# srv902/FOCUS

Measured on AMD Instinct MI355X. Metric: clips/sec (fwd+bwd+opt step) ORViT-MF 16x224, higher is better.
Workload: dtype bf16; 1 GPU; ORViT-Motionformer 16x224, 4 objects, batch=8 per GPU (BASELINE configs[1]); global_batch=8, frames=16, crop=224, objects=4, parallelism=dp1, optimizer=adamw+clipnorm

## Files before the change

### focus_amd/csrc/traj_time2_gw.hip

```cpp
#include "focus_common.h"
#include <algorithm>

namespace {

typedef __attribute__((ext_vector_type(8))) __bf16 bf16x8;
typedef __attribute__((ext_vector_type(4))) short s16x4;
typedef __attribute__((ext_vector_type(4))) float f32x4;
typedef __attribute__((address_space(3))) s16x4 lds_s16x4;

constexpr int HD = 64, TR = 32;
constexpr int C_ = 768;
constexpr int NSUB = C_ / 128;
constexpr int GT_BYTES = TR * C_ * 2, QT_BYTES = TR * HD * 2, STAGE = GT_BYTES + QT_BYTES;

union Frag { bf16x8 v; s16x4 t[2]; uint4 u; };

__device__ __forceinline__ int offb(int row, int ch) { return 256 * row + 16 * (ch ^ (((row & 3) << 2) | ((row >> 2) & 3))); }

__device__ __forceinline__ bf16x8 tr_frag_g(const char* sub, int r0, int c0, int lane) {
    const int i = lane & 15, q = i >> 2, p = i & 3;
    const int ch = (c0 >> 3) + (p >> 1), bo = 8 * (p & 1);
    Frag f;
    f.t[0] = __builtin_amdgcn_ds_read_tr16_b64_v4i16((lds_s16x4*)(sub + offb(r0 + q, ch) + bo));
    f.t[1] = __builtin_amdgcn_ds_read_tr16_b64_v4i16((lds_s16x4*)(sub + offb(r0 + 4 + q, ch) + bo));
    return f.v;
}
__device__ __forceinline__ bf16x8 tr_frag_q(const char* qt, int r0, int c0, int lane) {
    const int i = lane & 15, q = i >> 2, p = i & 3;
    const int o = (c0 + 4 * p) * 2;
    Frag f;
    f.t[0] = __builtin_amdgcn_ds_read_tr16_b64_v4i16((lds_s16x4*)(qt + (r0 + q) * 128 + o));
    f.t[1] = __builtin_amdgcn_ds_read_tr16_b64_v4i16((lds_s16x4*)(qt + (r0 + 4 + q) * 128 + o));
    return f.v;
}

__global__ __launch_bounds__(512) void time2_gw_kernel(const bf16_t* __restrict__ g, const bf16_t* __restrict__ q2,
                                                       const bf16_t* __restrict__ wk, int64_t wk_ld, bf16_t* __restrict__ dq2,
                                                       float* __restrict__ slabs, int R, int heads, int tiles_per_split) {
    extern __shared__ __attribute__((aligned(1024))) char smem[];
    const int h = blockIdx.y, sp = blockIdx.x;
    const int tid = threadIdx.x, lane = tid & 63, w = __builtin_amdgcn_readfirstlane(tid >> 6);
    const int ntiles_all = R / TR;
    const int t_begin = sp * tiles_per_split, t_end = min(ntiles_all, t_begin + tiles_per_split);
    const int row16_ = lane & 15, kq_ = lane >> 4;
    const int mb = w & 1, nbq = w >> 1;
    const bf16_t* gh = g + (int64_t)h * R * C_;

    bf16x8 wf[C_ / 32];
    {
        const bf16_t* wrow = wk + (int64_t)(h * HD + nbq * 16 + row16_) * wk_ld + kq_ * 8;
#pragma unroll
        for (int ks = 0; ks < C_ / 32; ++ks) wf[ks] = *reinterpret_cast<const bf16x8*>(wrow + ks * 32);
    }
    f32x4 accw[4][6];
#pragma unroll
    for (int a = 0; a < 4; ++a)
#pragma unroll
        for (int j = 0; j < 6; ++j) accw[a][j] = (f32x4){0.f, 0.f, 0.f, 0.f};
    asm volatile("s_waitcnt vmcnt(0)" ::: "memory");
#pragma unroll
    for (int ks = 0; ks < C_ / 32; ++ks) asm volatile("" : "+v"(wf[ks]));

    const uint32_t sm_a = lds_addr_of(smem);
    auto dma = [&](int t, int st) __attribute__((always_inline)) {
        const int64_t r0 = (int64_t)t * TR;
        const uint32_t base = sm_a + st * STAGE;
#pragma unroll
        for (int j = 0; j < 6; ++j) {
            const int p = w * 6 + j, sub = p >> 3, rg = p & 7;
            const int row = rg * 4 + (lane >> 4), pos = lane & 15;
            const int ch = pos ^ (((row & 3) << 2) | ((row >> 2) & 3));
            glds16(gh + (r0 + row) * C_ + sub * 128 + ch * 8, __builtin_amdgcn_readfirstlane(base + sub * 8192 + rg * 1024));
        }
        if (w < 4) {
            const int row = w * 8 + (lane >> 3);
            glds16(q2 + (r0 + row) * (int64_t)(heads * HD) + h * HD + (lane & 7) * 8,
                   __builtin_amdgcn_readfirstlane(base + GT_BYTES + w * 1024));
        }
    };
    if (t_begin >= t_end) return;
    dma(t_begin, 0);
    int st = 0;
    for (int t = t_begin; t < t_end; ++t) {
        const bool more = t + 1 < t_end;
        if (more) dma(t + 1, st ^ 1);
        if (more) { if (w < 4) asm volatile("s_waitcnt vmcnt(7)" ::: "memory"); else asm volatile("s_waitcnt vmcnt(6)" ::: "memory"); }
        else asm volatile("s_waitcnt vmcnt(0)" ::: "memory");
        __builtin_amdgcn_s_barrier();
        const char* gt = smem + st * STAGE;
        const char* qt = gt + GT_BYTES;
        int lane_o = lane;
        asm volatile("" : "+v"(lane_o));
        const int row16 = lane_o & 15, kq = lane_o >> 4;
        f32x4 accq = {0.f, 0.f, 0.f, 0.f};
#pragma unroll
        for (int ks = 0; ks < C_ / 32; ++ks) {
            const int col = ks * 32 + kq * 8;
            const bf16x8 af = *reinterpret_cast<const bf16x8*>(gt + (col >> 7) * 8192 + offb(mb * 16 + row16, (col & 127) >> 3));
            accq = __builtin_amdgcn_mfma_f32_16x16x32_bf16(af, wf[ks], accq, 0, 0, 0);
        }
        {
            bf16_t* o = dq2 + ((int64_t)t * TR + mb * 16 + kq * 4) * (heads * HD) + h * HD + nbq * 16 + row16;
#pragma unroll
            for (int r = 0; r < 4; ++r) o[(int64_t)r * (heads * HD)] = f32_to_bf16(accq[r]);
        }
#pragma unroll
        for (int j = 0; j < 6; ++j) {
            const int c = w * 96 + j * 16;
            const bf16x8 gb = tr_frag_g(gt + (c >> 7) * 8192, 8 * kq, c & 127, lane_o);
#pragma unroll
            for (int a = 0; a < 4; ++a) {
                const bf16x8 qa = tr_frag_q(qt, 8 * kq, a * 16, lane_o);
                accw[a][j] = __builtin_amdgcn_mfma_f32_16x16x32_bf16(qa, gb, accw[a][j], 0, 0, 0);
            }
        }
        asm volatile("s_waitcnt lgkmcnt(0)" ::: "memory");
        __builtin_amdgcn_s_barrier();
        st ^= 1;
    }
    float* out = slabs + ((int64_t)sp * heads * HD + h * HD) * C_;
#pragma unroll
    for (int a = 0; a < 4; ++a)
#pragma unroll
        for (int j = 0; j < 6; ++j)
#pragma unroll
            for (int r = 0; r < 4; ++r) out[(int64_t)(a * 16 + kq_ * 4 + r) * C_ + w * 96 + j * 16 + row16_] = accw[a][j][r];
}

__global__ __launch_bounds__(256) void time2_gw_reduce_kernel(const float* __restrict__ slabs, float* __restrict__ dwk, int64_t n4,
                                                              int splits) {
    const int64_t i = (int64_t)blockIdx.x * 256 + threadIdx.x;
    if (i >= n4) return;
    float4 s = reinterpret_cast<const float4*>(slabs)[i];
#pragma unroll 4
    for (int k = 1; k < splits; ++k) {
        const float4 v = reinterpret_cast<const float4*>(slabs)[(int64_t)k * n4 + i];
        s.x += v.x; s.y += v.y; s.z += v.z; s.w += v.w;
    }
    reinterpret_cast<float4*>(dwk)[i] = s;
}

int gw_splits(int R, int heads) {
    const int tiles = R / TR;
    return std::max(1, std::min(tiles, 256 / std::max(heads, 1)));
}

}

extern "C" int focus_traj_time2_gw_ok(int R, int heads, int d, int dtype) {
    return dtype == FOCUS_BF16 && d == HD && heads * d == C_ && R >= TR && R % TR == 0;
}

extern "C" size_t focus_traj_time2_gw_workspace_bytes(int R, int heads, int d) {
    if (!focus_traj_time2_gw_ok(R, heads, d, FOCUS_BF16)) return 0;
    return (size_t)gw_splits(R, heads) * C_ * C_ * sizeof(float);
}

extern "C" int focus_traj_time2_gw(const void* g, const void* q2, const void* wk, int64_t wk_ld, void* dq2, float* dwk, void* ws,
                                   size_t ws_bytes, int R, int heads, int d, int dtype, void* stream) {
    if (!g || !q2 || !wk || !dq2 || !dwk || !ws) return FOCUS_ERR_NULL;
    if (!focus_traj_time2_gw_ok(R, heads, d, dtype) || (wk_ld & 7)) return FOCUS_ERR_SHAPE;
    if (!focus_aligned(g, 16) || !focus_aligned(q2, 16) || !focus_aligned(wk, 16) || !focus_aligned(dwk, 16)) return FOCUS_ERR_ALIGN;
    if (ws_bytes < focus_traj_time2_gw_workspace_bytes(R, heads, d)) return FOCUS_ERR_WORKSPACE;
    hipStream_t s = static_cast<hipStream_t>(stream);
    const int splits = gw_splits(R, heads), tiles = R / TR;
    const int tps = (tiles + splits - 1) / splits;
    const int used = (tiles + tps - 1) / tps;
    auto k = time2_gw_kernel;
    const size_t lds = 2 * (size_t)STAGE;
    static bool once = (hipFuncSetAttribute((const void*)k, hipFuncAttributeMaxDynamicSharedMemorySize, lds) == hipSuccess);
    (void)once;
    hipLaunchKernelGGL(k, dim3(used, heads), dim3(512), lds, s, (const bf16_t*)g, (const bf16_t*)q2, (const bf16_t*)wk, wk_ld,
                       (bf16_t*)dq2, (float*)ws, R, heads, tps);
    FOCUS_CHECK_LAUNCH();
    const int64_t n4 = (int64_t)C_ * C_ / 4;
    hipLaunchKernelGGL(time2_gw_reduce_kernel, dim3((unsigned)cdiv64(n4, 256)), dim3(256), 0, s, (const float*)ws, dwk, n4, used);
    FOCUS_CHECK_LAUNCH();
    return FOCUS_OK;
}
```

### focus_amd/ops.py

```python
import ctypes
import weakref

import torch

from . import _lib
from ._lib import BF16, F32, GemmDesc

EPI_NONE, EPI_GELU, EPI_RELU, EPI_TANH = _lib.EPI_NONE, _lib.EPI_GELU, _lib.EPI_RELU, _lib.EPI_TANH
_DEPI = {EPI_GELU: _lib.EPI_DGELU, EPI_RELU: _lib.EPI_DRELU, EPI_TANH: _lib.EPI_DTANH}


def _dt(t):
    if t.dtype == torch.float32:
        return F32
    if t.dtype == torch.bfloat16:
        return BF16
    raise RuntimeError("focus_amd: unsupported dtype %s (float32 or bfloat16)" % t.dtype)


def _need_gpu(*ts):
    for t in ts:
        if t is not None and not t.is_cuda:
            raise RuntimeError("focus_amd: the hot path runs on the MI355X only (got a %s tensor); "
                               "there is no CPU fallback" % t.device)
# ... 1157 lines not shown
    def backward(ctx, dxt, dxdiag, dcls):
        qkv, xt, cls_out, lse, cls_lse = ctx.saved_tensors
        B, F_, P, heads, d = ctx.dims
        dxt, dxdiag, dcls = dxt.contiguous(), dxdiag.contiguous(), dcls.contiguous()
        dqkv = torch.empty_like(qkv)
        L = _lib.lib()
        nb = L.focus_traj_space_workspace_bytes(B, F_, P, heads, d, _dt(qkv), 1)
        ws = torch.empty(max(nb, 16), device=qkv.device, dtype=torch.uint8)
        _lib.check(L.focus_traj_space_bwd(_p(qkv), _p(xt), _p(cls_out), _p(lse), _p(cls_lse), _p(dxt), _p(dxdiag),
                                          _p(dcls), _p(dqkv), _p(ws), nb, B, F_, P, heads, d, _dt(qkv), _stream()),
                   "traj_space_bwd")
        return dqkv, None, None, None


def traj_space(qkv, F_, P, heads):
    return _TrajSpaceFn.apply(qkv, F_, P, heads)


class _TrajTimeFn(torch.autograd.Function):
    @staticmethod
    def forward(ctx, q2, k2, xt, heads):
        _need_gpu(q2, k2, xt)
        q2, k2, xt = q2.contiguous(), k2.contiguous(), xt.contiguous()
        B, S, F_, C = xt.shape
        d = C // heads
        out = torch.empty(B, S, C, device=xt.device, dtype=xt.dtype)
        attn2 = torch.empty(B, heads, S, F_, device=xt.device, dtype=torch.float32)
        _lib.check(_lib.lib().focus_traj_time_fwd(_p(q2), _p(k2), _p(xt), _p(out), S * C, _p(attn2), B, S, F_, heads, d,
                                                  _dt(xt), _stream()), "traj_time_fwd")
        ctx.save_for_backward(q2, k2, xt, attn2)
        ctx.heads = heads
        return out

    @staticmethod
    def backward(ctx, dout):
        q2, k2, xt, attn2 = ctx.saved_tensors
        B, S, F_, C = xt.shape
        dout = dout.contiguous()
        dq2, dk2, dxt = torch.empty_like(q2), torch.empty_like(k2), torch.empty_like(xt)
        _lib.check(_lib.lib().focus_traj_time_bwd(_p(q2), _p(k2), _p(xt), _p(attn2), _p(dout), S * C, _p(dq2), _p(dk2),
                                                  _p(dxt), 0, B, S, F_, ctx.heads, C // ctx.heads, _dt(xt),
                                                  _stream()), "traj_time_bwd")
        return dq2, dk2, dxt, None


def traj_time(q2, k2, xt, heads):
    return _TrajTimeFn.apply(q2, k2, xt, heads)


class _TrajTimeBlockFn(torch.autograd.Function):

    @staticmethod
    def forward(ctx, q2, xt, w_kv, b_kv, cls_out, heads):
        _need_gpu(q2, xt, w_kv)
        q2, xt = q2.contiguous(), xt.contiguous()
        B, S, F_, C = xt.shape
        d = C // heads
        wk = shadow(w_kv, xt.dtype)[:C]
        bk = b_kv.detach()[:C] if b_kv is not None else None
        k2 = mm_nt(xt.view(-1, C), wk, bias=bk).view(B, S, F_, C)
        out = torch.empty(B, S + 1, C, device=xt.device, dtype=xt.dtype)
        out[:, 0].copy_(cls_out.reshape(B, C))
        attn2 = torch.empty(B, heads, S, F_, device=xt.device, dtype=torch.float32)
        _lib.check(_lib.lib().focus_traj_time_fwd(_p(q2), _p(k2), _p(xt), _p(out, C), (S + 1) * C, _p(attn2), B, S, F_,
                                                  heads, d, _dt(xt), _stream()), "traj_time_fwd")
        ctx.save_for_backward(q2, k2, xt, attn2, w_kv)
        ctx.heads, ctx.has_b, ctx.cls_shape = heads, b_kv is not None, cls_out.shape
        return out

    @staticmethod
    def backward(ctx, dcat):
        q2, k2, xt, attn2, w_kv = ctx.saved_tensors
        B, S, F_, C = xt.shape
        dcat = dcat.contiguous()
        dq2, dk2, dxt_a = torch.empty_like(q2), torch.empty_like(k2), torch.empty_like(xt)
        _lib.check(_lib.lib().focus_traj_time_bwd(_p(q2), _p(k2), _p(xt), _p(attn2), _p(dcat, C), (S + 1) * C, _p(dq2),
                                                  _p(dk2), _p(dxt_a), 0, B, S, F_, ctx.heads, C // ctx.heads, _dt(xt),
                                                  _stream()), "traj_time_bwd")
        dk2f, xt2 = dk2.view(-1, C), xt.view(-1, C)
        dw = db = dwk = dbk = None
        join = None
        if ctx.needs_input_grad[2]:
            dwk, dbk, join = wgrad_async(dk2f, xt2, ctx.has_b and ctx.needs_input_grad[3])
        dxt = None
        if ctx.needs_input_grad[1]:
            if xt.dtype == torch.bfloat16 and C % 64 == 0:
                wt = shadow(w_kv, xt.dtype, transposed=True)
                dxt = mm_nt(dk2f, wt[:, :C], residual=dxt_a.view(-1, C))
            else:
                dxt = mm_nn(dk2f, shadow(w_kv, xt.dtype)[:C]).add_(dxt_a.view(-1, C))
            dxt = dxt.view(B, S, F_, C)
        if join is not None:
            join()
        if dwk is not None:
            dw = torch.empty(2 * C, C, device=xt.device, dtype=torch.float32)
            dw[:C].copy_(dwk)
            dw[C:].zero_()
            if dbk is not None:
                db = torch.zeros(2 * C, device=xt.device, dtype=torch.float32)
                db[:C].copy_(dbk)
        dcls = dcat[:, :1].reshape(ctx.cls_shape) if ctx.needs_input_grad[4] else None
        return dq2, dxt, dw, db, dcls, None


def traj_time_block(q2, xt, w_kv, b_kv, cls_out, heads):
    return _TrajTimeBlockFn.apply(q2, xt, w_kv, b_kv, cls_out, heads)


class _TrajTime2BlockFn(torch.autograd.Function):

    @staticmethod
    def forward(ctx, q2, xt, w_kv, b_kv, cls_out, heads):
        _need_gpu(q2, xt, w_kv)
        q2, xt = q2.contiguous(), xt.contiguous()
        B, S, F_, C = xt.shape
        d = C // heads
        L = _lib.lib()
        wkT = shadow(w_kv, xt.dtype, transposed=True)
        out = torch.empty(B, S + 1, C, device=xt.device, dtype=xt.dtype)
        out[:, 0].copy_(cls_out.reshape(B, C))
        attn2 = torch.empty(B, S, heads, F_, device=xt.device, dtype=torch.float32)
        nb = L.focus_traj_time2_workspace_bytes(B, S, F_, heads, d)
        ws = torch.empty(nb // 4, device=xt.device, dtype=torch.float32)
        _lib.check(L.focus_traj_time2_fwd(_p(q2), _p(xt), _p(wkT), wkT.stride(0), _p(out, C), (S + 1) * C, _p(attn2),
                                          _p(ws), nb, B, S, F_, heads, d, _dt(xt), _stream()), "traj_time2_fwd")
        ctx.save_for_backward(q2, xt, attn2, w_kv)
        ctx.heads, ctx.has_b, ctx.cls_shape = heads, b_kv is not None, cls_out.shape
        return out

    @staticmethod
    def backward(ctx, dcat):
        q2, xt, attn2, w_kv = ctx.saved_tensors
        heads = ctx.heads
        B, S, F_, C = xt.shape
        d = C // heads
        dev = xt.device
        L = _lib.lib()
        dcat = dcat.contiguous()
        wkT = shadow(w_kv, xt.dtype, transposed=True)
        dxt = torch.empty_like(xt)
        g = torch.empty(heads, B * S, C, device=dev, dtype=xt.dtype)
        dl = torch.empty(B, S, F_, 16, device=dev, dtype=xt.dtype)
        _lib.check(L.focus_traj_time2_bwd(_p(q2), _p(xt), _p(wkT), wkT.stride(0), _p(attn2), _p(dcat, C), (S + 1) * C,
                                          _p(dxt), _p(g), _p(dl), B, S, F_, heads, d, _dt(xt), _stream()), "traj_time2_bwd")
        R = B * S
        dq2 = dw = db = None
        if (ctx.needs_input_grad[0] and ctx.needs_input_grad[2] and L.focus_traj_time2_gw_ok(R, heads, d, _dt(xt))
                and _os.environ.get("FOCUS_TIME2_GW", "1") != "0"):
            wk = shadow(w_kv, xt.dtype)
            dq2 = torch.empty(B, S, C, device=dev, dtype=xt.dtype)
            dw = torch.empty(2 * C, C, device=dev, dtype=torch.float32)
            nbw = L.focus_traj_time2_gw_workspace_bytes(R, heads, d)
            wsw = torch.empty(nbw // 4, device=dev, dtype=torch.float32)
            _lib.check(L.focus_traj_time2_gw(_p(g), _p(q2), _p(wk), wk.stride(0), _p(dq2), _p(dw), _p(wsw), nbw, R, heads, d,
                                             _dt(xt), _stream()), "traj_time2_gw")
            dw[C:].zero_()
            if ctx.has_b and ctx.needs_input_grad[3]:
                db = torch.zeros(2 * C, device=dev, dtype=torch.float32)
            dcls = dcat[:, :1].reshape(ctx.cls_shape) if ctx.needs_input_grad[4] else None
            return dq2, dxt, dw, db, dcls, None
        if ctx.needs_input_grad[0]:
            wk = shadow(w_kv, xt.dtype)
            dq2 = torch.empty(B, S, C, device=dev, dtype=xt.dtype)
            gemm(R, d, C, (g, 0), (C, 1, 0, R * C), (wk, 0), (1, C, 0, d * C), (dq2, 0), (C, 1, 0, d),
                 batch=(1, heads))
        if ctx.needs_input_grad[2]:
            dw = torch.empty(2 * C, C, device=dev, dtype=torch.float32)
            nbw = L.focus_gemm_tn_batched_workspace_bytes(d, C, R, heads)
            wsw = torch.empty(max(nbw, 16) // 4, device=dev, dtype=torch.float32)
            gemm(d, C, R, (q2, 0), (1, C, 0, d), (g, 0), (C, 1, 0, R * C), (dw, 0), (C, 1, 0, d * C),
                 batch=(1, heads), aux=(wsw, 0))
            dw[C:].zero_()
            if ctx.has_b and ctx.needs_input_grad[3]:
                db = torch.zeros(2 * C, device=dev, dtype=torch.float32)
        dcls = dcat[:, :1].reshape(ctx.cls_shape) if ctx.needs_input_grad[4] else None
        return dq2, dxt, dw, db, dcls, None


def traj_time2_ok(xt, heads):
    if _os.environ.get("FOCUS_TIME2", "1") == "0" or xt.dtype != torch.bfloat16:
        return False
    B, S, F_, C = xt.shape
    return C % heads == 0 and C // heads == 64 and heads <= 16 and F_ in (4, 8, 16)


def traj_time2_block(q2, xt, w_kv, b_kv, cls_out, heads):
    return _TrajTime2BlockFn.apply(q2, xt, w_kv, b_kv, cls_out, heads)


class _SmallAttnFn(torch.autograd.Function):

    @staticmethod
    def forward(ctx, q, k, v, heads, scale, causal, drop):
        _need_gpu(q, k, v)
        B, N, C = q.shape
        M = k.shape[1]
        d = C // heads
        dev, dt = q.device, q.dtype
        att = torch.empty(B, heads, N, M, device=dev, dtype=dt)
        L = _lib.lib()
        ctx.heads, ctx.scale = heads, scale

        def rows_ok(t):
            return t.stride(2) == 1 and t.stride(0) == t.shape[1] * t.stride(1) and t.stride(1) >= C

        ctx.fused = (not causal and drop is None and bool(L.focus_small_attn_ok(N, M, d))
                     and rows_ok(q) and rows_ok(k) and rows_ok(v))
        if ctx.fused:
            out = torch.empty(B, N, C, device=dev, dtype=dt)
            _lib.check(L.focus_small_attn_fwd(_p(q), _p(k), _p(v), q.stride(1), k.stride(1), v.stride(1), _p(att), _p(out), B,
                                              heads, N, M, d, scale, _dt(q), _stream()), "small_attn_fwd")
            ctx.save_for_backward(q, k, v, att, None)
            return out
        q, k, v = q.contiguous(), k.contiguous(), v.contiguous()
        sa = (M, 1, heads * N * M, N * M)
        gemm(N, M, d, (q, 0), (C, 1, N * C, d), (k, 0), (1, C, M * C, d), (att, 0), sa, batch=(B, heads))
        if causal:
            assert N == M, "causal self-attention"
            _lib.check(L.focus_softmax_causal_fwd(_p(att), _p(att), B * heads * N, M, M, N, scale, _dt(att), _stream()),
                       "softmax_causal_fwd")
        else:
            _lib.check(L.focus_softmax_fwd(_p(att), _p(att), B * heads * N, M, M, scale, _dt(att), _stream()),
                       "softmax_fwd")
        attd = att if drop is None else att * drop
        out = torch.empty(B, N, C, device=dev, dtype=dt)
        gemm(N, d, M, (attd, 0), sa, (v, 0), (C, 1, M * C, d), (out, 0), (C, 1, N * C, d), batch=(B, heads))
        ctx.save_for_backward(q, k, v, att, drop)
        return out

    @staticmethod
    def backward(ctx, dout):
        q, k, v, att, drop = ctx.saved_tensors
        heads, scale = ctx.heads, ctx.scale
        B, N, C = q.shape
        M = k.shape[1]
        d = C // heads
        dout = dout.contiguous()
        if ctx.fused:
            es = q.element_size()
            if (N == M and q.stride(1) == 3 * C == k.stride(1) == v.stride(1) and k.data_ptr() == q.data_ptr() + C * es
                    and v.data_ptr() == k.data_ptr() + C * es):
                dqkv = torch.empty(B, N, 3 * C, device=q.device, dtype=q.dtype)
                dq, dk, dv = dqkv[..., :C], dqkv[..., C:2 * C], dqkv[..., 2 * C:]
            else:
                dq = torch.empty(q.shape, device=q.device, dtype=q.dtype)
                dk = torch.empty(k.shape, device=q.device, dtype=q.dtype)
                dv = torch.empty(v.shape, device=q.device, dtype=q.dtype)
                if not (q.is_contiguous() and k.is_contiguous() and v.is_contiguous()):
                    q, k, v = q.contiguous(), k.contiguous(), v.contiguous()
            _lib.check(_lib.lib().focus_small_attn_bwd(_p(q), _p(k), _p(v), q.stride(1), k.stride(1), v.stride(1), _p(att),
                                                       _p(dout), _p(dq), _p(dk), _p(dv), B, heads, N, M, d, scale, _dt(q),
                                                       _stream()), "small_attn_bwd")
            return dq, dk, dv, None, None, None, None
        sa = (M, 1, heads * N * M, N * M)
        sat = (1, M, heads * N * M, N * M)
        sq = (C, 1, N * C, d)
        sk = (C, 1, M * C, d)
        attd = att if drop is None else att * drop
        datt = torch.empty_like(att)
        gemm(N, M, d, (dout, 0), sq, (v, 0), (1, C, M * C, d), (datt, 0), sa, batch=(B, heads))
        dv = torch.empty_like(v)
        gemm(M, d, N, (attd, 0), sat, (dout, 0), sq, (dv, 0), sk, batch=(B, heads))
        if drop is not None:
            datt = datt * drop
        _lib.check(_lib.lib().focus_softmax_bwd(_p(datt), _p(att), _p(datt), B * heads * N, M, M, scale, _dt(att),
                                                _stream()), "softmax_bwd")
        dq, dk = torch.empty_like(q), torch.empty_like(k)
        gemm(N, d, M, (datt, 0), sa, (k, 0), sk, (dq, 0), sq, batch=(B, heads))
        gemm(M, d, N, (datt, 0), sat, (q, 0), sq, (dk, 0), sk, batch=(B, heads))
        return dq, dk, dv, None, None, None, None


def flash_ok(q, k, v, heads, causal):
    if not (q.is_cuda and q.dtype == torch.bfloat16 and k.dtype == q.dtype and v.dtype == q.dtype and q.dim() == 3):
        return False
    C = q.shape[2]
    if C % heads:
        return False
    for t in (q, k, v):
        if t.stride(2) != 1 or t.stride(1) % 8 or t.stride(0) % 8 or t.data_ptr() % 16:
            return False
    return bool(_lib.lib().focus_flash_attn_ok(q.shape[1], k.shape[1], C // heads, _lib.BF16, int(bool(causal))))


def drop_threshold(p):
    thr = int(round(float(p) * 65536.0))
    assert 0 <= thr < 65536, "dropout probability out of range"
    return thr


def _flash_args(q, k, v, out, lse, heads, scale, causal, thr, seed):
    B, Nq, C = q.shape
    a = _lib.FlashArgs()
    a.q, a.k, a.v, a.out, a.lse = _p(q), _p(k), _p(v), _p(out), _p(lse)
    a.seed = _p(seed) if seed is not None else None
    a.ldq, a.ldk, a.ldv, a.ldo = q.stride(1), k.stride(1), v.stride(1), out.stride(1)
    a.bsq, a.bsk, a.bsv, a.bso = q.stride(0), k.stride(0), v.stride(0), out.stride(0)
    a.B, a.heads, a.Nq, a.Nk, a.d, a.dtype, a.causal = B, heads, Nq, k.shape[1], C // heads, _lib.BF16, int(bool(causal))
    a.drop_thr, a.scale = thr, scale
    return a


class _FlashAttnFn(torch.autograd.Function):

    @staticmethod
    def forward(ctx, q, k, v, heads, scale, causal, thr, seed):
        _need_gpu(q, k, v)
        B, Nq, C = q.shape
        out = torch.empty(B, Nq, C, device=q.device, dtype=q.dtype)
        lse = torch.empty(B, heads, Nq, device=q.device, dtype=torch.float32)
        a = _flash_args(q, k, v, out, lse, heads, scale, causal, thr, seed)
# ... 989 lines not shown
```

### include/focus_amd.h

```cpp
#ifndef FOCUS_AMD_H
#define FOCUS_AMD_H

#include <stddef.h>
#include <stdint.h>

#ifdef __cplusplus
extern "C" {
#endif

enum focus_dtype { FOCUS_F32 = 0, FOCUS_BF16 = 1, FOCUS_FP8_E4M3 = 2  };

enum focus_status {
    FOCUS_OK = 0,
    FOCUS_ERR_SHAPE = -1,
    FOCUS_ERR_DTYPE = -2,
    FOCUS_ERR_ALIGN = -3,
    FOCUS_ERR_LAUNCH = -4,
    FOCUS_ERR_NULL = -5,
    FOCUS_ERR_WORKSPACE = -6
};

const char* focus_strerror(int status);
int focus_abi_version(void);

// ... 102 lines not shown

int focus_roi_align_fwd(const void* feat, int64_t img_stride, int imgs_per_batch, int64_t batch_stride,
                        const float* rois, const int32_t* roi_img, void* out, int NI, int C, int H, int W, int K,
                        int PH, int PW, float spatial_scale, int sampling_ratio, int aligned, int relu, int dtype,
                        void* stream);
size_t focus_roi_align_bwd_workspace_bytes(int NI, int C, int H, int W, int PH, int PW);
int focus_roi_align_bwd(const void* dout, const void* relu_out, const float* rois, const int32_t* roi_img, void* dfeat, int64_t img_stride,
                        int imgs_per_batch, int64_t batch_stride, void* ws, size_t ws_bytes, int NI, int C, int H, int W, int K, int PH, int PW, float spatial_scale,
                        int sampling_ratio, int aligned, int dtype, void* stream);
int focus_roi_align_indices(const float* rois, int32_t* grid, int32_t* nbr, int H, int W, int K, int PH,
                            int PW, float spatial_scale, int sampling_ratio, int aligned, void* stream);

int focus_cell_amax_fwd(const void* x, void* y, int32_t* arg, int K, int cells, int C, int dtype,
                        void* stream);
int focus_cell_amax_bwd(const void* dy, const int32_t* arg, void* dx, int K, int cells, int C, int dtype,
                        void* stream);

int focus_orvit_assemble(const void* x, const void* obj, void* all, int B, int T, int HW, int O, int C, int dtype,
                         void* stream);
int focus_orvit_assemble_bwd(const void* dall, void* dx, void* dobj, int B, int T, int HW, int O, int C, int dtype,
                             void* stream);
int focus_orvit_merge(const void* x, const void* y, const void* mm, const float* scale, void* out, int B, int T, int HW,
                      int O, int C, int dtype, void* stream);
int focus_orvit_merge_bwd(const void* dout, const float* scale, void* dy, void* dmm, int B, int T, int HW, int O, int C,
                          int dtype, void* stream);

int focus_box_layout_fwd(const void* vecs, const float* boxes, void* out, int NF, int O, int C, int H,
                         int W, int dtype, void* stream);
int focus_box_layout_bwd(const void* dout, const float* boxes, void* dvecs, int NF, int O, int C, int H,
                         int W, int dtype, void* stream);

size_t focus_slot_attn_workspace_bytes(int B, int N, int K, int D);
int focus_slot_attn_fwd(const void* k_t, const void* v_t, int64_t kv_bstride, const void* q, void* attn_vis,
                        int64_t attn_bstride, void* upd, float* colsum, void* partial, size_t partial_bytes,
                        int B, int N, int K, int D, float eps, int dtype, void* stream);
int focus_slot_attn_bwd(const void* k_t, const void* v_t, int64_t kv_bstride, const void* q,
                        const void* attn_vis, int64_t attn_bstride, const float* colsum, const void* upd,
                        const void* dupd,
                        const void* dattn_vis, void* dk_t, void* dv_t, int accumulate, void* dq, void* partial,
                        size_t partial_bytes, int B, int N, int K, int D, float eps, int dtype, void* wl, void* stream);
int focus_slot_kv_grad_ok(int K, int D, int dtype, int iters);
int focus_slot_kv_grad(const void* wl0, const void* wl1, const void* wl2, const void* wl3, const void* q0, const void* q1,
                       const void* q2, const void* q3, const void* du0, const void* du1, const void* du2, const void* du3,
                       int iters, void* dk_t, void* dv_t, int64_t kv_bstride, int64_t kv_ld, int B, int N, int K, int D,
                       int dtype, void* stream);

int focus_small_attn_ok(int N, int M, int d);
int focus_small_attn_fwd(const void* q, const void* k, const void* v, int64_t ldq, int64_t ldk, int64_t ldv, void* att,
                         void* out, int B, int heads, int N, int M, int d, float scale, int dtype, void* stream);
int focus_small_attn_bwd(const void* q, const void* k, const void* v, int64_t ldq, int64_t ldk, int64_t ldv, const void* att,
                         const void* dout, void* dq, void* dk, void* dv, int B, int heads, int N, int M, int d, float scale,
                         int dtype, void* stream);

int focus_gru_gates_fwd(void* gi, void* gh, const void* h, void* hn, const float* b_ih, const float* b_hh, int R, int D,
                        int dtype, void* stream);
int focus_gru_gates_bwd(const void* gi, const void* gh, const void* h, const void* dhn, void* dgi, void* dgh,
                        void* dh, void* zero_out, int R, int D, int dtype, void* stream);

int focus_im2col_patches(const float* x, void* cols, int B, int Cin, int T, int H, int W, int kt, int kh,
                         int kw, int dtype, void* stream);

int focus_embed_assemble(const void* patch, const float* cls, const float* pos, const float* temp,
                         void* tokens, int B, int T, int P, int C, int dtype, void* stream);

int focus_xent_ls(const float* logits, const int64_t* target, float* loss_rows, float* dlogits, int R,
                  int Ncls, float smoothing, void* stream);

int focus_transpose_pad(const void* src, int src_dtype, int64_t src_ld, int64_t src_bstride, void* dst,
                        int dst_dtype, int64_t dst_ld, int64_t dst_bstride, int R, int Cc, int batch,
                        void* stream);

typedef struct focus_shadow_item {
    const float* src; void* dst; void* dstT;
    int32_t rows, cols;
} focus_shadow_item;
int focus_shadow_refresh(const focus_shadow_item* items, int n_items, int max_rows, int max_cols, void* stream);

typedef struct focus_adamw_item {
    float* p; float* m; float* v; void* dst; void* dstT;
    int32_t rows, cols, group, unit0, tile_mode, pad_;
} focus_adamw_item;
int focus_adamw_units(int rows, int cols, int tile_mode);
size_t focus_adamw_workspace_bytes(void);
int focus_adamw_step(const focus_adamw_item* items, float* const* grads, int n_items, int n_units, const float* groups, float* steps,
                     void* workspace, size_t workspace_bytes, float* total_norm, double beta1, double beta2, float eps,
                     float max_norm, int write_clipped_grads, void* stream);

typedef struct focus_fp8_item {
    const float* src; void* dst; void* dstT; float* scale;
    int32_t rows, cols;
} focus_fp8_item;
int focus_fp8_refresh(const focus_fp8_item* items, int n_items, int max_rows, int max_cols, void* amax_scratch, void* stream);

typedef struct focus_wgrad_item {
    const void* dy; const void* x; float* dw; float* db;
    int64_t ld_dy, ld_x;
    int32_t M, N, K, pad_;
} focus_wgrad_item;
int focus_linear_wgrad_group_units(const focus_wgrad_item* items, int n_items);
int focus_linear_wgrad_group_plan(const focus_wgrad_item* items, int n_items, void* host_units, size_t bytes);
int focus_linear_wgrad_group(const focus_wgrad_item* items, int n_items, const void* dev_units, void* stream);

typedef struct focus_slot_tail_args {
    int32_t R, D, H, do_gru, do_mlp, do_q;
    float ln1_eps, ln2_eps;
    const void* upd; const void* h;
    const void* w_ih; const void* w_hh; const float* b_ih; const float* b_hh;
    const float* ln1_g; const float* ln1_b; const void* w1; const float* b1; const void* w2; const float* b2;
    const float* ln2_g; const float* ln2_b; const void* wq;
    void* g; void* hn; void* y; float* mean1; float* rstd1; void* a; void* s;
    void* sn; float* mean2; float* rstd2; void* q;
} focus_slot_tail_args;
int focus_slot_tail_ok(int D, int H, int dtype);
int focus_slot_tail_fwd(const focus_slot_tail_args* args, void* stream);
typedef struct focus_slot_tail_bwd_args {
    int32_t R, D, H, do_gru, do_mlp, do_q;
    const void* dout; const void* dq;
    const void* h; const void* g; const void* hn; const void* a; const void* cur;
    const float* mean1; const float* rstd1; const float* mean2; const float* rstd2;
    const float* ln1_g; const float* ln2_g;
    const void* w_ih_t; const void* w_hh_t; const void* w1_t; const void* w2_t; const void* wq_t;
    void* dupd; void* dh; void* ds; void* dz; void* dg; float* part1; float* part2;
    void* ws_dsn; void* ws_dy1; void* ws_res;
} focus_slot_tail_bwd_args;
int focus_slot_tail_bwd_blocks(int R);
int focus_slot_tail_bwd(const focus_slot_tail_bwd_args* args, void* stream);

typedef struct focus_flash_args {
    const void* q; const void* k; const void* v; void* out; float* lse;
    const void* dout; float* delta; void* dq; void* dk; void* dv;
    const uint32_t* seed;
    int64_t ldq, ldk, ldv, ldo, lddo, lddq, lddk, lddv;
    int64_t bsq, bsk, bsv, bso, bsdo, bsdq, bsdk, bsdv;
    int32_t B, heads, Nq, Nk, d, dtype, causal;
    uint32_t drop_thr;
    float scale;
    int32_t pad_;
} focus_flash_args;
int focus_flash_attn_ok(int Nq, int Nk, int d, int dtype, int causal);
int focus_flash_attn_fwd(const focus_flash_args* args, void* stream);
int focus_flash_attn_bwd(const focus_flash_args* args, void* stream);

int focus_decode_attn_ok(int Lmax, int d, int dtype);
int focus_decode_attn(const void* q, int64_t ldq, const void* k_new, const void* v_new, int64_t ldn, void* k_cache,
                      void* v_cache, int64_t ldc, int64_t bsc, void* out, int64_t ldo, int B, int heads, int d, int len,
                      int Lmax, float scale, int dtype, void* stream);
int focus_greedy_next(const void* logits, int64_t ldl, const float* dict, const float* pe_row, int64_t* tok,
                      int64_t tok_stride, void* x_next, int64_t ldx, int B, int V, int D, int dtype, void* stream);

int focus_traj_time2_gw_ok(int R, int heads, int d, int dtype);
size_t focus_traj_time2_gw_workspace_bytes(int R, int heads, int d);
int focus_traj_time2_gw(const void* g, const void* q2, const void* wk, int64_t wk_ld, void* dq2, float* dwk, void* ws,
                        size_t ws_bytes, int R, int heads, int d, int dtype, void* stream);

int focus_rows_ok(int64_t R, int V, int dtype);
int focus_gumbel_fwd(const void* x, const float* e_soft, const float* e_hard, const void* seed, void* z, int64_t* target,
                     float* stats, int64_t R, int V, float tau, int hard, int dtype, int dtype_z, void* stream);
int focus_gumbel_bwd(const void* x, const float* e_soft, const void* seed, const float* stats, const void* dz, void* dx,
                     int64_t R, int V, float tau, int dtype, int dtype_z, void* stream);

int focus_xent_rows_fwd(const void* logits, const int64_t* target, float* loss_rows, float* lse, int64_t R, int V,
                        float smoothing, int dtype, void* stream);
int focus_xent_rows_bwd(const void* logits, const int64_t* target, const float* lse, const float* g, void* dlogits,
                        int64_t R, int V, float smoothing, int dtype, void* stream);

int focus_dropout_add(const void* y, const void* res, const void* seed, int thr, void* out, int64_t n, int dtype,
                      void* stream);

int focus_diag_gather(const void* xt, void* xdiag, int B, int S, int F, int C, int dtype, void* stream);
int focus_diag_scatter_add(const void* dxdiag, void* dxt, int B, int S, int F, int C, int dtype, void* stream);

int focus_scale_add(const void* x, const void* y, const float* scale, float keep, void* out, int B, int64_t per,
                    int dtype, void* stream);

int focus_cast(const void* src, int src_dtype, void* dst, int dst_dtype, int64_t n, void* stream);

#ifdef __cplusplus
}
#endif
#endif
```

Before: 285.9 clips/s.

## Split dq K-reduction across waves via LDS and fuse dW/db zeroing into reduce

The time2 grad-weight kernel now splits the dq2 GEMM over two K halves per wave pair, keeping half the weight fragments in registers. Partial sums go to an LDS buffer and are reduced and stored as vectorized bf16 by the other waves one tile later. MFMA and LDS reads are interleaved with sched_group_barriers, and the q fragments are hoisted out of the dW loop. A new _full entry point makes the reduce kernel also zero the second half of dW and the bias gradient, replacing two separate torch zero launches, at the cost of extra LDS, an extra lgkmcnt wait per tile, and more complex synchronization.

```diff
diff --git a/focus_amd/csrc/traj_time2_gw.hip b/focus_amd/csrc/traj_time2_gw.hip
--- a/focus_amd/csrc/traj_time2_gw.hip
+++ b/focus_amd/csrc/traj_time2_gw.hip
@@ -12,6 +12,9 @@
 constexpr int C_ = 768;
 constexpr int NSUB = C_ / 128;
 constexpr int GT_BYTES = TR * C_ * 2, QT_BYTES = TR * HD * 2, STAGE = GT_BYTES + QT_BYTES;
+constexpr int KH = C_ / 64;
+constexpr int DQ_BYTES = 2 * TR * HD * 4;
+constexpr int RD_AHEAD = 8;
 
 union Frag { bf16x8 v; s16x4 t[2]; uint4 u; };
 
@@ -43,14 +46,14 @@
     const int ntiles_all = R / TR;
     const int t_begin = sp * tiles_per_split, t_end = min(ntiles_all, t_begin + tiles_per_split);
     const int row16_ = lane & 15, kq_ = lane >> 4;
-    const int mb = w & 1, nbq = w >> 1;
+    const int kh = w & 1, nbq = w >> 1;
     const bf16_t* gh = g + (int64_t)h * R * C_;
 
-    bf16x8 wf[C_ / 32];
+    bf16x8 wf[KH];
     {
-        const bf16_t* wrow = wk + (int64_t)(h * HD + nbq * 16 + row16_) * wk_ld + kq_ * 8;
-#pragma unroll
-        for (int ks = 0; ks < C_ / 32; ++ks) wf[ks] = *reinterpret_cast<const bf16x8*>(wrow + ks * 32);
+        const bf16_t* wrow = wk + (int64_t)(h * HD + nbq * 16 + row16_) * wk_ld + kh * (C_ / 2) + kq_ * 8;
+#pragma unroll
+        for (int ks = 0; ks < KH; ++ks) wf[ks] = *reinterpret_cast<const bf16x8*>(wrow + ks * 32);
     }
     f32x4 accw[4][6];
 #pragma unroll
@@ -59,7 +62,7 @@
         for (int j = 0; j < 6; ++j) accw[a][j] = (f32x4){0.f, 0.f, 0.f, 0.f};
     asm volatile("s_waitcnt vmcnt(0)" ::: "memory");
 #pragma unroll
-    for (int ks = 0; ks < C_ / 32; ++ks) asm volatile("" : "+v"(wf[ks]));
+    for (int ks = 0; ks < KH; ++ks) asm volatile("" : "+v"(wf[ks]));
 
     const uint32_t sm_a = lds_addr_of(smem);
     auto dma = [&](int t, int st) __attribute__((always_inline)) {
@@ -77,6 +80,18 @@
             glds16(q2 + (r0 + row) * (int64_t)(heads * HD) + h * HD + (lane & 7) * 8,
                    __builtin_amdgcn_readfirstlane(base + GT_BYTES + w * 1024));
         }
+    };
+    float* dqs = reinterpret_cast<float*>(smem + 2 * STAGE);
+    const int fin_row = ((w & 3) * 64 + lane) >> 3, fin_c8 = (lane & 7) * 8;
+    auto dq_sum = [&](float (&v)[8]) __attribute__((always_inline)) {
+        const float4* p0 = reinterpret_cast<const float4*>(dqs + fin_row * HD + fin_c8);
+        const float4* p1 = p0 + TR * HD / 4;
+        const float4 a0 = p0[0], a1 = p0[1], b0 = p1[0], b1 = p1[1];
+        v[0] = a0.x + b0.x; v[1] = a0.y + b0.y; v[2] = a0.z + b0.z; v[3] = a0.w + b0.w;
+        v[4] = a1.x + b1.x; v[5] = a1.y + b1.y; v[6] = a1.z + b1.z; v[7] = a1.w + b1.w;
+    };
+    auto dq_store = [&](int t, const float (&v)[8]) __attribute__((always_inline)) {
+        st8<bf16_t>(dq2 + ((int64_t)t * TR + fin_row) * (heads * HD) + h * HD + fin_c8, v);
     };
     if (t_begin >= t_end) return;
     dma(t_begin, 0);
@@ -84,40 +99,66 @@
     for (int t = t_begin; t < t_end; ++t) {
         const bool more = t + 1 < t_end;
         if (more) dma(t + 1, st ^ 1);
+        const bool fin = w >= 4 && t > t_begin;
+        float dv[8];
+        if (fin) dq_sum(dv);
         if (more) { if (w < 4) asm volatile("s_waitcnt vmcnt(7)" ::: "memory"); else asm volatile("s_waitcnt vmcnt(6)" ::: "memory"); }
         else asm volatile("s_waitcnt vmcnt(0)" ::: "memory");
+        if (fin) dq_store(t - 1, dv);
+        asm volatile("s_waitcnt lgkmcnt(0)" ::: "memory");
         __builtin_amdgcn_s_barrier();
+        asm volatile("" ::: "memory");
         const char* gt = smem + st * STAGE;
         const char* qt = gt + GT_BYTES;
         int lane_o = lane;
         asm volatile("" : "+v"(lane_o));
         const int row16 = lane_o & 15, kq = lane_o >> 4;
-        f32x4 accq = {0.f, 0.f, 0.f, 0.f};
-#pragma unroll
-        for (int ks = 0; ks < C_ / 32; ++ks) {
-            const int col = ks * 32 + kq * 8;
-            const bf16x8 af = *reinterpret_cast<const bf16x8*>(gt + (col >> 7) * 8192 + offb(mb * 16 + row16, (col & 127) >> 3));
-            accq = __builtin_amdgcn_mfma_f32_16x16x32_bf16(af, wf[ks], accq, 0, 0, 0);
-        }
+        __builtin_amdgcn_sched_barrier(0);
+        f32x4 accq[2] = {{0.f, 0.f, 0.f, 0.f}, {0.f, 0.f, 0.f, 0.f}};
+#pragma unroll
+        for (int ks = 0; ks < KH; ++ks) {
+            const int col = kh * (C_ / 2) + ks * 32 + kq * 8;
+#pragma unroll
+            for (int mb = 0; mb < 2; ++mb) {
+                const bf16x8 af = *reinterpret_cast<const bf16x8*>(gt + (col >> 7) * 8192 + offb(mb * 16 + row16, (col & 127) >> 3));
+                accq[mb] = __builtin_amdgcn_mfma_f32_16x16x32_bf16(af, wf[ks], accq[mb], 0, 0, 0);
+            }
+        }
+        __builtin_amdgcn_sched_group_barrier(0x100, RD_AHEAD, 0);
+#pragma unroll
+        for (int i = 0; i < 2 * KH - RD_AHEAD; ++i) {
+            __builtin_amdgcn_sched_group_barrier(0x008, 1, 0);
+            __builtin_amdgcn_sched_group_barrier(0x100, 1, 0);
+        }
+        __builtin_amdgcn_sched_group_barrier(0x008, RD_AHEAD, 0);
+        __builtin_amdgcn_sched_barrier(0);
         {
-            bf16_t* o = dq2 + ((int64_t)t * TR + mb * 16 + kq * 4) * (heads * HD) + h * HD + nbq * 16 + row16;
-#pragma unroll
-            for (int r = 0; r < 4; ++r) o[(int64_t)r * (heads * HD)] = f32_to_bf16(accq[r]);
-        }
+            float* o = dqs + kh * (TR * HD) + (kq * 4) * HD + nbq * 16 + row16;
+#pragma unroll
+            for (int mb = 0; mb < 2; ++mb)
+#pragma unroll
+                for (int r = 0; r < 4; ++r) o[(mb * 16 + r) * HD] = accq[mb][r];
+        }
+        bf16x8 qa[4];
+#pragma unroll
+        for (int a = 0; a < 4; ++a) qa[a] = tr_frag_q(qt, 8 * kq, a * 16, lane_o);
 #pragma unroll
         for (int j = 0; j < 6; ++j) {
             const int c = w * 96 + j * 16;
             const bf16x8 gb = tr_frag_g(gt + (c >> 7) * 8192, 8 * kq, c & 127, lane_o);
 #pragma unroll
-            for (int a = 0; a < 4; ++a) {
-                const bf16x8 qa = tr_frag_q(qt, 8 * kq, a * 16, lane_o);
-                accw[a][j] = __builtin_amdgcn_mfma_f32_16x16x32_bf16(qa, gb, accw[a][j], 0, 0, 0);
-            }
+            for (int a = 0; a < 4; ++a) accw[a][j] = __builtin_amdgcn_mfma_f32_16x16x32_bf16(qa[a], gb, accw[a][j], 0, 0, 0);
         }
         asm volatile("s_waitcnt lgkmcnt(0)" ::: "memory");
         __builtin_amdgcn_s_barrier();
+        asm volatile("" ::: "memory");
         st ^= 1;
     }
+    if (w >= 4) {
+        float dv[8];
+        dq_sum(dv);
+        dq_store(t_end - 1, dv);
+    }
     float* out = slabs + ((int64_t)sp * heads * HD + h * HD) * C_;
 #pragma unroll
     for (int a = 0; a < 4; ++a)
@@ -127,10 +168,18 @@
             for (int r = 0; r < 4; ++r) out[(int64_t)(a * 16 + kq_ * 4 + r) * C_ + w * 96 + j * 16 + row16_] = accw[a][j][r];
 }
 
+template <bool FULL>
 __global__ __launch_bounds__(256) void time2_gw_reduce_kernel(const float* __restrict__ slabs, float* __restrict__ dwk, int64_t n4,
-                                                              int splits) {
+                                                              int splits, float* __restrict__ db, int ndb4) {
     const int64_t i = (int64_t)blockIdx.x * 256 + threadIdx.x;
-    if (i >= n4) return;
+    if (i >= n4) {
+        if (FULL) {
+            const float4 z = make_float4(0.f, 0.f, 0.f, 0.f);
+            if (i < 2 * n4) reinterpret_cast<float4*>(dwk)[i] = z;
+            else if (db && i - 2 * n4 < ndb4) reinterpret_cast<float4*>(db)[i - 2 * n4] = z;
+        }
+        return;
+    }
     float4 s = reinterpret_cast<const float4*>(slabs)[i];
 #pragma unroll 4
     for (int k = 1; k < splits; ++k) {
@@ -156,25 +205,47 @@
     return (size_t)gw_splits(R, heads) * C_ * C_ * sizeof(float);
 }
 
-extern "C" int focus_traj_time2_gw(const void* g, const void* q2, const void* wk, int64_t wk_ld, void* dq2, float* dwk, void* ws,
-                                   size_t ws_bytes, int R, int heads, int d, int dtype, void* stream) {
-    if (!g || !q2 || !wk || !dq2 || !dwk || !ws) return FOCUS_ERR_NULL;
+namespace {
+
+int gw_launch(const void* g, const void* q2, const void* wk, int64_t wk_ld, void* dq2, float* dw, float* db, bool full, void* ws,
+              size_t ws_bytes, int R, int heads, int d, int dtype, void* stream) {
+    if (!g || !q2 || !wk || !dq2 || !dw || !ws) return FOCUS_ERR_NULL;
     if (!focus_traj_time2_gw_ok(R, heads, d, dtype) || (wk_ld & 7)) return FOCUS_ERR_SHAPE;
-    if (!focus_aligned(g, 16) || !focus_aligned(q2, 16) || !focus_aligned(wk, 16) || !focus_aligned(dwk, 16)) return FOCUS_ERR_ALIGN;
+    if (!focus_aligned(g, 16) || !focus_aligned(q2, 16) || !focus_aligned(wk, 16) || !focus_aligned(dq2, 16) ||
+        !focus_aligned(dw, 16) || !focus_aligned(ws, 16) || (db && !focus_aligned(db, 16)))
+        return FOCUS_ERR_ALIGN;
     if (ws_bytes < focus_traj_time2_gw_workspace_bytes(R, heads, d)) return FOCUS_ERR_WORKSPACE;
     hipStream_t s = static_cast<hipStream_t>(stream);
     const int splits = gw_splits(R, heads), tiles = R / TR;
     const int tps = (tiles + splits - 1) / splits;
     const int used = (tiles + tps - 1) / tps;
     auto k = time2_gw_kernel;
-    const size_t lds = 2 * (size_t)STAGE;
+    const size_t lds = 2 * (size_t)STAGE + DQ_BYTES;
     static bool once = (hipFuncSetAttribute((const void*)k, hipFuncAttributeMaxDynamicSharedMemorySize, lds) == hipSuccess);
     (void)once;
     hipLaunchKernelGGL(k, dim3(used, heads), dim3(512), lds, s, (const bf16_t*)g, (const bf16_t*)q2, (const bf16_t*)wk, wk_ld,
                        (bf16_t*)dq2, (float*)ws, R, heads, tps);
     FOCUS_CHECK_LAUNCH();
     const int64_t n4 = (int64_t)C_ * C_ / 4;
-    hipLaunchKernelGGL(time2_gw_reduce_kernel, dim3((unsigned)cdiv64(n4, 256)), dim3(256), 0, s, (const float*)ws, dwk, n4, used);
+    const int ndb4 = 2 * C_ / 4;
+    if (full)
+        hipLaunchKernelGGL(time2_gw_reduce_kernel<true>, dim3((unsigned)cdiv64(2 * n4 + ndb4, 256)), dim3(256), 0, s,
+                           (const float*)ws, dw, n4, used, db, ndb4);
+    else
+        hipLaunchKernelGGL(time2_gw_reduce_kernel<false>, dim3((unsigned)cdiv64(n4, 256)), dim3(256), 0, s, (const float*)ws, dw,
+                           n4, used, (float*)nullptr, 0);
     FOCUS_CHECK_LAUNCH();
     return FOCUS_OK;
 }
+
+}
+
+extern "C" int focus_traj_time2_gw(const void* g, const void* q2, const void* wk, int64_t wk_ld, void* dq2, float* dwk, void* ws,
+                                   size_t ws_bytes, int R, int heads, int d, int dtype, void* stream) {
+    return gw_launch(g, q2, wk, wk_ld, dq2, dwk, nullptr, false, ws, ws_bytes, R, heads, d, dtype, stream);
+}
+
+extern "C" int focus_traj_time2_gw_full(const void* g, const void* q2, const void* wk, int64_t wk_ld, void* dq2, float* dw,
+                                        float* db, void* ws, size_t ws_bytes, int R, int heads, int d, int dtype, void* stream) {
+    return gw_launch(g, q2, wk, wk_ld, dq2, dw, db, true, ws, ws_bytes, R, heads, d, dtype, stream);
+}
diff --git a/focus_amd/ops.py b/focus_amd/ops.py
--- a/focus_amd/ops.py
+++ b/focus_amd/ops.py
@@ -1333,11 +1333,10 @@
             dw = torch.empty(2 * C, C, device=dev, dtype=torch.float32)
             nbw = L.focus_traj_time2_gw_workspace_bytes(R, heads, d)
             wsw = torch.empty(nbw // 4, device=dev, dtype=torch.float32)
-            _lib.check(L.focus_traj_time2_gw(_p(g), _p(q2), _p(wk), wk.stride(0), _p(dq2), _p(dw), _p(wsw), nbw, R, heads, d,
-                                             _dt(xt), _stream()), "traj_time2_gw")
-            dw[C:].zero_()
             if ctx.has_b and ctx.needs_input_grad[3]:
-                db = torch.zeros(2 * C, device=dev, dtype=torch.float32)
+                db = torch.empty(2 * C, device=dev, dtype=torch.float32)
+            _lib.check(L.focus_traj_time2_gw_full(_p(g), _p(q2), _p(wk), wk.stride(0), _p(dq2), _p(dw), _p(db), _p(wsw), nbw, R,
+                                                  heads, d, _dt(xt), _stream()), "traj_time2_gw_full")
             dcls = dcat[:, :1].reshape(ctx.cls_shape) if ctx.needs_input_grad[4] else None
             return dq2, dxt, dw, db, dcls, None
         if ctx.needs_input_grad[0]:
diff --git a/include/focus_amd.h b/include/focus_amd.h
--- a/include/focus_amd.h
+++ b/include/focus_amd.h
@@ -278,6 +278,8 @@
 size_t focus_traj_time2_gw_workspace_bytes(int R, int heads, int d);
 int focus_traj_time2_gw(const void* g, const void* q2, const void* wk, int64_t wk_ld, void* dq2, float* dwk, void* ws,
                         size_t ws_bytes, int R, int heads, int d, int dtype, void* stream);
+int focus_traj_time2_gw_full(const void* g, const void* q2, const void* wk, int64_t wk_ld, void* dq2, float* dw, float* db,
+                             void* ws, size_t ws_bytes, int R, int heads, int d, int dtype, void* stream);
 
 int focus_rows_ok(int64_t R, int V, int dtype);
 int focus_gumbel_fwd(const void* x, const float* e_soft, const float* e_hard, const void* seed, void* z, int64_t* target,
```

Measured after the change: 287.8 clips/s, median of 4. No clear change (+0.7%).
